# Sir-Teo/MuZero-Go

Hardware: AMD Instinct MI355X
Metric: MCTS simulations/sec (whole node) + self-play moves/sec, 9x9 Go, 200 sims/move (higher is better)
Workload: dtype fp32

## Files before the change

### muzero-go_amd/csrc/mzgo_capi.hip

```cpp
#include <hip/hip_runtime.h>

#include <algorithm>
#include <cmath>
#include <cstdarg>
#include <cstdio>
#include <cstring>
#include <map>
#include <string>
#include <vector>

#include "../../include/mzgo.h"
#include "mzgo_dispatch.hpp"
#include "mzgo_replay.hpp"
#include "mzgo_tower_host.hpp"
#include "mzgo_weights.hpp"

namespace mzgo {
extern const KernelSet kernels_n5_c96, kernels_n6_c96, kernels_n9_c96, kernels_n19_c96, kernels_n6_c128,
    kernels_n6_c64;

const KernelSet* find_kernels(int N, int C) {
  static const KernelSet* all[] = {&kernels_n5_c96, &kernels_n6_c96, &kernels_n9_c96, &kernels_n19_c96,
                                   &kernels_n6_c128, &kernels_n6_c64};
  for (const KernelSet* k : all)
// ... 38 lines not shown
  std::string key;
  std::vector<int64_t> shape;
};

std::vector<Spec> specs(int C, int A) {
  std::vector<Spec> out;
  for (int k = 0; k < WK_COUNT; ++k) {
    const WeightShape sh = weight_key_shape(k, C, A);
    out.push_back(Spec{kWeightKeyNames[k], std::vector<int64_t>(sh.d, sh.d + sh.nd)});
  }
  return out;
}

}

static int device_cus() {
  static int ncu[64];
  int dev = 0;
  if (hipGetDevice(&dev) != hipSuccess || dev < 0 || dev >= 64) return 0;
  if (ncu[dev] <= 0) {
    int n = 0;
    if (hipDeviceGetAttribute(&n, hipDeviceAttributeMultiprocessorCount, dev) != hipSuccess) n = 0;
    ncu[dev] = n;
  }
  return ncu[dev];
}

struct mzgo_engine {
  mzgo_config cfg;
  const KernelSet* ks = nullptr;
  int N = 0, C = 0, A = 0, CELLS = 0, CS = 0, G = 0, S = 0, M = 0;
  int TS = 0;
  std::map<std::string, std::vector<float>> sd;
  std::vector<Spec> spec;
  bool dirty = true;
  bool dev_weights = false;
  WeightLayout wl;
  float* d_w = nullptr;
  size_t d_w_bytes = 0;
  NetParams np{};
  EngineArrays E{};
  int* d_err = nullptr;
  unsigned* rq_head = nullptr;
  float* d_scr = nullptr;
  size_t scr_floats = 0;
  std::vector<void*> allocs;
  bool timing = false;
  std::vector<hipEvent_t> tev;
  int tn = 0;
  int64_t bytes = 0;
  int epoch = 0;
  int value_cache = 0;
  int arrival_conv = 1;
  const double* noise = nullptr;
  double* noise_out = nullptr;
  TowerHost* tower = nullptr;

  template <class T>
  int alloc(T** p, size_t n) {
    void* v = nullptr;
    hipError_t e = hipMalloc(&v, n * sizeof(T) + 256);
    if (e != hipSuccess) return fail(MZGO_EHIP, "hipMalloc(%zu): %s", n * sizeof(T), hipGetErrorString(e));
    allocs.push_back(v);
    bytes += (int64_t)(n * sizeof(T));
    *p = reinterpret_cast<T*>(v);
    return MZGO_OK;
  }
  ~mzgo_engine() {
    if (tower) {
      for (hipEvent_t ev : tower->evs) (void)hipEventDestroy(ev);
      tower->free_chains();
      for (void* p : {tower->d_wb, (void*)tower->d_wf, (void*)tower->ib, (void*)tower->ob, (void*)tower->s0,
                      (void*)tower->s1, (void*)tower->shp, (void*)tower->sact})
        if (p) (void)hipFree(p);
      if (tower->h_total) (void)hipHostFree(tower->h_total);
      tower->free_batch();
      delete tower;
    }
    for (hipEvent_t ev : tev) (void)hipEventDestroy(ev);
    for (void* p : allocs) (void)hipFree(p);
    if (d_w) (void)hipFree(d_w);
    if (d_scr) (void)hipFree(d_scr);
  }

  int ensure_blob() {
    if (d_w) return MZGO_OK;
    wl = weight_layout(N, C, A);
    HIPCHK(hipMalloc(&d_w, wl.total * 4));
    d_w_bytes = wl.total * 4;
    HIPCHK(hipMemset(d_w, 0, d_w_bytes));
    const float* b = d_w;
    const size_t* off = wl.off;
    np.w_conv1 = b + off[WP_CONV1_W]; np.b_conv1 = b + off[WP_CONV1_B];
    np.w_conv2 = b + off[WP_CONV2_W]; np.b_conv2 = b + off[WP_CONV2_B];
    np.w_conv3 = b + off[WP_CONV3_W]; np.b_conv3 = b + off[WP_CONV3_B];
    np.w_dyn = b + off[WP_DYN_W]; np.b_dyn = b + off[WP_DYN_B];
    np.emb = b + off[WP_EMB]; np.head_w = b + off[WP_HEAD_W]; np.etab = b + off[WP_ETAB];
    np.hs.reward_b = b + off[WP_REWARD_B]; np.hs.fc1_w = b + off[WP_FC1_W]; np.hs.fc1_b = b + off[WP_FC1_B];
    np.hs.fc2_w = b + off[WP_FC2_W]; np.hs.fc2_b = b + off[WP_FC2_B]; np.hs.value_b = b + off[WP_VALUE_B];
    np.hs.vfc_w = b + off[WP_VFC_W]; np.hs.vfc_b = b + off[WP_VFC_B]; np.hs.policy_b = b + off[WP_POLICY_B];
    np.hs.pass_logit = b + off[WP_PASS_LOGIT];
    return MZGO_OK;
  }

  int sync_weights() {
    if (C == 0) return fail(MZGO_EINVAL, "board-only engine (latent_dim 0) has no network");
    if (!dirty) return MZGO_OK;
    for (const Spec& s : spec)
      if (!sd.count(s.key)) return fail(MZGO_ENOWEIGHTS, "missing weight '%s'", s.key.c_str());
    if (tower) {
      HIPCHK(tower->upload(sd));
      dirty = false;
      return MZGO_OK;
    }
    if (int rc = ensure_blob()) return rc;
    const float* src[WK_COUNT];
    for (int k = 0; k < WK_COUNT; ++k) src[k] = sd[spec[k].key].data();
    std::vector<float> blob(wl.total, 0.f);
    pack_weights_host(wl, src, blob.data());
    HIPCHK(hipMemcpy(d_w, blob.data(), wl.total * 4, hipMemcpyHostToDevice));
    dev_weights = false;
    dirty = false;
    return MZGO_OK;
  }

  int tower_scratch(int B) {
    TowerHost& t = *tower;
    if (B <= t.scap) return MZGO_OK;
    for (void* p : {(void*)t.ib, (void*)t.ob, (void*)t.s0, (void*)t.s1, (void*)t.shp, (void*)t.sact})
      if (p) HIPCHK(hipFree(p));
    t.ib = t.ob = t.s0 = t.s1 = nullptr; t.shp = nullptr; t.sact = nullptr; t.scap = 0;
    const size_t n = (size_t)B * t.slot();
    for (bf16** q : {&t.ib, &t.ob, &t.s0, &t.s1}) {
      HIPCHK(hipMalloc((void**)q, n * sizeof(bf16)));
      HIPCHK(hipMemset(*q, 0, n * sizeof(bf16)));
    }
    HIPCHK(hipMalloc((void**)&t.shp, (size_t)B * t.CC * 3 * t.CS * sizeof(float)));
    HIPCHK(hipMalloc((void**)&t.sact, (size_t)B * sizeof(int)));
    t.scap = B;
    return MZGO_OK;
  }

  SearchParams search_params() const {
    SearchParams sp;
    sp.c_puct = cfg.c_puct; sp.discount = cfg.discount;
    sp.dirichlet_alpha = cfg.dirichlet_alpha; sp.dirichlet_epsilon = cfg.dirichlet_epsilon;
    sp.pass_epsilon = cfg.pass_epsilon; sp.num_simulations = S; sp.compat = cfg.compat;
    sp.variant = cfg.search_variant;
    sp.factored = cfg.direct_dynamics ? 0 : 1;
    sp.seed = cfg.seed;
    sp.helpers = 0;
    sp.net = 0;
    sp.tail = 0;
    const char* lz = getenv("MZGO_LAZY_ROWS");
    sp.lazy_rows = lz && atoi(lz) == 0 ? 0 : 1;
    sp.value_cache = value_cache;
    sp.arrival_conv = arrival_conv;
    sp.fast_simulations = 0;
    sp.full_search_prob = 1.0;
    return sp;
  }
  SearchParams selfplay_params() const {
    SearchParams sp = search_params();
    if (!tower && cfg.full_search_prob < 1.0) {
      sp.fast_simulations = cfg.fast_simulations;
      sp.full_search_prob = cfg.full_search_prob;
    }
    return sp;
  }
};

void mzgo::replay_engine_view(const mzgo_engine* e, ReplayEngineView* v) {
  const EngineArrays& E = e->E;
  *v = ReplayEngineView{e->N, e->G, e->M, e->C, e->tower ? 1 : 0, e->cfg.game_base, e->epoch,
                        E.stones, E.invd, E.meta, E.rec_stones, E.rec_invd, E.rec_flags, E.rec_action,
                        E.rec_value, E.rec_policy, E.rec_reward, E.final_reward};
}

extern "C" {

const char* mzgo_last_error(void) { return g_err.c_str(); }

void mzgo_default_config(mzgo_config* c, int N) {
  std::memset(c, 0, sizeof *c);
  c->board_size = N;
  c->latent_dim = 96;
  c->num_games = 1;
  c->num_simulations = 128;
  c->max_moves = N * N;
  c->compat = 0;
  c->temperature_moves = 15;
  c->c_puct = 2.5;
  c->discount = 0.99;
  c->dirichlet_alpha = 0.15;
  c->dirichlet_epsilon = 0.02;
  c->pass_epsilon = 0.01;
  c->temperature = 1.0;
  c->komi = 0.0;
  c->seed = 1234;
  c->fast_simulations = 0;
  c->full_search_prob = 1.0;
}

int mzgo_playout_budget_host(uint64_t seed, uint32_t key_gid, int move, int num_simulations, int fast_simulations,
                             double full_search_prob, int* budget) {
  if (!budget) return fail(MZGO_EINVAL, "mzgo_playout_budget_host: null budget");
  if (num_simulations < 1 || move < 0)
    return fail(MZGO_EINVAL, "mzgo_playout_budget_host: num_simulations %d must be >= 1 and move %d >= 0",
                num_simulations, move);
  if (fast_simulations < 0 || fast_simulations > num_simulations)
// ... 86 lines not shown
    T.bq_cap = t->bq_cap;
    chk(e->alloc(&T.pool, G * n1 * slot));
    chk(e->alloc(&t->t0, G * slot));
    chk(e->alloc(&t->t1, G * slot));
    chk(e->alloc(&T.rep_in, G * (size_t)t->P * 64));
    if (rc == MZGO_OK) {
      for (auto pr : {std::make_pair((void*)T.pool, G * n1 * slot), std::make_pair((void*)t->t0, G * slot),
                      std::make_pair((void*)t->t1, G * slot), std::make_pair((void*)T.rep_in, G * (size_t)t->P * 64)})
        if (hipMemset(pr.first, 0, pr.second * sizeof(bf16)) != hipSuccess) chk(fail(MZGO_EHIP, "hipMemset(tower) failed"));
    }
    T.slot = (long long)slot;
    chk(e->alloc(&T.hpart, G * (size_t)t->CC * 3 * e->CS));
    chk(e->alloc(&T.bq_n, G));
    chk(e->alloc(&T.bq_nid0, G));
    chk(e->alloc(&T.nbg, G));
    chk(e->alloc(&T.b_total, 1));
    if (rc == MZGO_OK && (hipMemset(T.bq_n, 0, G * sizeof(int)) != hipSuccess ||
                          hipHostMalloc(&t->h_total, sizeof(int), hipHostMallocDefault) != hipSuccess))
      chk(fail(MZGO_EHIP, "tower batch setup failed"));
    chk(e->alloc(&T.rootmask, G * A));
    chk(e->alloc(&T.passp, G));
    chk(e->alloc(&T.key, G));
    chk(e->alloc(&T.playing, G));
    chk(e->alloc(&T.evalact, G));
    chk(e->alloc(&T.in_idx, G));
    chk(e->alloc(&T.out_idx, G));
    chk(e->alloc(&T.root_idx, G));
    chk(e->alloc(&T.act, G));
    chk(e->alloc(&T.job, G * 3));
    chk(e->alloc(&T.simc, G));
    if (rc == MZGO_OK) {
      std::vector<int> ri(G);
      for (size_t g = 0; g < G; ++g) ri[g] = (int)(g * n1);
      if (hipMemcpy(T.root_idx, ri.data(), G * sizeof(int), hipMemcpyHostToDevice) != hipSuccess ||
          hipMemset(T.playing, 0, G * sizeof(int)) != hipSuccess || hipMemset(T.evalact, 0, G * sizeof(int)) != hipSuccess)
        chk(fail(MZGO_EHIP, "tower index setup failed"));
    }
  }
  if (C != 0) {
    chk(e->alloc(&E.prior, TSL * n1 * A));
    chk(e->alloc(&E.child, TSL * n1 * A));
    chk(e->alloc(&E.visits, TSL * n1));
    chk(e->alloc(&E.wsum, TSL * n1));
    chk(e->alloc(&E.root_prior, TSL * A));
    chk(e->alloc(&E.path, TSL * (n1 + 1)));
    chk(e->alloc(&E.nodes, TSL));
    chk(e->alloc(&E.nact, TSL * n1));
    const char* vc = getenv("MZGO_VALUE_CACHE");
    e->value_cache = !TW && !cfg->direct_dynamics && ks->value_cache_cap > 0 && e->S + 2 <= ks->value_cache_cap &&
                     !(vc && atoi(vc) == 0);
    if (e->value_cache) chk(e->alloc(&E.cval, TSL * n1 * A));
    const char* ac = getenv("MZGO_ARRIVAL_CONV");
    e->arrival_conv = !(ac && atoi(ac) <= 0);
    chk(e->alloc(&E.jobs, TSL * job_bytes(A)));
    chk(e->alloc(&E.mpq, 2 * (size_t)G + 1));
    chk(e->alloc(&E.rec_stones, G * M * CELLS));
    chk(e->alloc(&E.rec_invd, G * M * CELLS));
    chk(e->alloc(&E.rec_flags, G * M));
    chk(e->alloc(&E.rec_action, G * M));
    chk(e->alloc(&E.rec_value, G * M));
    chk(e->alloc(&E.rec_policy, G * M * A));
    chk(e->alloc(&E.rec_reward, G * M));
  }
  chk(e->alloc(&E.stones, G * CELLS));
  chk(e->alloc(&E.invd, G * CELLS));
  chk(e->alloc(&E.meta, G * 4));
  chk(e->alloc(&E.game_len, G));
  chk(e->alloc(&E.final_reward, G));
  chk(e->alloc(&E.status, G));
  chk(e->alloc(&E.counters, kCounters));
  chk(e->alloc(&e->d_err, 1));
  chk(e->alloc(&e->rq_head, 1));
#ifdef MZGO_STAMPS
  chk(e->alloc(&E.stamps, TSL * kStampPhases));
  if (E.stamps) (void)hipMemset(E.stamps, 0, TSL * kStampPhases * 8);
#endif
  if (rc != MZGO_OK) { delete e; return rc; }
  if (hipMemset(E.counters, 0, kCounters * sizeof(unsigned long long)) != hipSuccess ||
      hipMemset(e->d_err, 0, sizeof(int)) != hipSuccess) {
    delete e;
    return fail(MZGO_EHIP, "hipMemset failed");
  }
  hipError_t he = ks->board_reset(E, e->G, nullptr);
  if (he == hipSuccess) he = hipDeviceSynchronize();
  if (he != hipSuccess) { delete e; return fail(MZGO_EHIP, "board reset: %s", hipGetErrorString(he)); }
  *out = e;
  return MZGO_OK;
}

void mzgo_engine_destroy(mzgo_engine* e) { delete e; }

int64_t mzgo_engine_device_bytes(const mzgo_engine* e) { return e ? e->bytes + (int64_t)e->d_w_bytes : 0; }

int mzgo_set_weights(mzgo_engine* e, const char* key, const float* data, const int64_t* shape, int ndim) {
  if (!e || !key || !data || (!shape && ndim > 0)) return fail(MZGO_EINVAL, "null argument");
  for (const Spec& s : e->spec) {
    if (s.key != key) continue;
    if ((int)s.shape.size() != ndim) return fail(MZGO_EINVAL, "'%s': expected %zu dims, got %d", key, s.shape.size(), ndim);
    size_t n = 1;
    for (int i = 0; i < ndim; ++i) {
      if (shape[i] != s.shape[i])
        return fail(MZGO_EINVAL, "'%s': dim %d is %lld, expected %lld", key, i, (long long)shape[i], (long long)s.shape[i]);
      n *= (size_t)shape[i];
    }
    e->sd[key].assign(data, data + n);
    e->dirty = true;
// ... 578 lines not shown
```

### muzero-go_amd/csrc/mzgo_kernels.hpp

```cpp
#pragma once
#include "mzgo_jobs.hpp"
#include "mzgo_replay.hpp"

namespace mzgo {

template <class G>
constexpr bool rep_needs_scratch() {
  if constexpr (G::WINO) return Wino<G>::NSTRIP > 1;
  else return false;
}

struct NoRepJobs {
  __device__ bool operator()(int) const { return false; }
};

template <class G, class PlaneFn, class Jobs = NoRepJobs>
__device__ __forceinline__ void representation(Smem<G>& sm, const NetParams& np, PlaneFn planes, float* lat,
                                      int lat_stride, float* scr, unsigned long long* ts = nullptr,
                                      Jobs jobs = Jobs{}) {
  float* mid = rep_needs_scratch<G>() ? scr : lat;
  for (int i = tid_local(); i < 6 * G::CELLS; i += G::THREADS) {
    const int c = i / G::CELLS, j = i - c * G::CELLS;
    sm.u.in[c * G::CPAD + j] = planes(c, j);
  }
// ... 400 lines not shown
    if (y_lds_target<G>(sm) != nullptr && !shared_jobs<G>(sp)) load_hw<G>(sm, np.head_w);
    else load_y<G>(sm, pool, np.head_w);
    if (tid_local() == 0) { sm.t.npick = 0; sm.t.ngrab = 0; }
    __syncthreads();
    if (st) st->lap(61);
    if (shared_jobs<G>(sp)) {
      batch_expand_shared<G, Acc::LDS>(sm, np, sp, E, g, TV, K, 1, 0, sp.net, pool, el, n, 0, key, 0, nullptr, true);
    } else {
      if (wave_id() == 0) pick_sequence<G>(el, n, 0, K, key, 0, L.acts, &sm.t.npick, G::WAVES);
      batch_expand<G, Acc::LDS>(sm, np, sp, TV, K, 1, pool, st);
    }
    __syncthreads();
    if (st) st->lap(62);
    if (wave_id() == 0) {
      const int lane = lane_id_local();
      for (int k = lane; k < K; k += 64) {
        const int a = L.acts[k], nid = 1 + k;
        const double v = L.bv[k];
        T.init(nid);
        T.add(nid, v);
        T.set_child(0, a, nid);
        T.add_root_child(a, v);
        nact[nid] = a;
      }
      if (lane == 0) {
        const bool alt = sp.variant == 0;
        const double wroot = prefix_sums<G>(T.ws(0), L.bv, K, alt, nullptr);
        T.set(0, T.vis(0) + K, wroot);
        sm.t.newest = -1;
        sm.t.ycache = 0;
      }
    }
    __syncthreads();
    return K;
  }
}

template <class G, int DMAX>
struct VerifyLds {
  double cP[DMAX][64 * G::AP];
  double q[DMAX][64 * G::AP];
  double inv1n[DMAX][64 * G::AP];
  int n[DMAX][64 * G::AP];
  double qx[DMAX][G::A + 1], invr[DMAX][G::A + 1], sq[DMAX][G::A + 1], sx[DMAX][G::A + 1];
  uint64_t elig[DMAX][G::AP];
  double lo_o[DMAX], hi_o[DMAX];
  double cpx[DMAX];
  int x[DMAX], n0[DMAX], N0[DMAX];
  double wpre[DMAX][G::A + 9];
  double wroot[G::A + 9];
  uint64_t failm[G::AP];
  uint64_t exactm[DMAX][G::AP];
  int fail;
};
template <class G>
constexpr int verify_depth() { return G::AP > 2 ? 2 : 8; }
constexpr int kSeqK = 16, kSharedSeqK = 32;
__device__ __forceinline__ bool replay_sequential(int B, int depth) { return (B - 1) * (depth + 1) < kSeqK; }
__device__ __forceinline__ bool replay_parallel(bool shared, int B, int depth) {
  if (shared) return (B - 1) * (depth + 1) >= kSharedSeqK;
  return !replay_sequential(B, depth);
}

template <class G, class Acc, class V>
__device__ __forceinline__ void verify_load_level(Smem<G>& sm, const SearchParams& sp, const TreeView& TV,
                                                  const Acc& T, const int* nact, V& vl, int k, int l, int ract) {
  const int lane = lane_id_local();
  const int p = T.path(l);
  const int xa = l == 0 ? ract : nact[T.path(l + 1)];
  double lo = INFINITY, hi = -INFINITY, cpx = 0.0;
  int nx = 0;
#pragma unroll
  for (int j = 0; j < G::AP; ++j) {
    const int a = lane + 64 * j;
    const bool in = a < G::A;
    double P, w = 0.0;
    int n = 0;
    if (l == 0) {
      P = in ? T.root_prior(a) : 0.0;
      if constexpr (Acc::LDS) {
        if (in) { n = sm.t.rvis[a]; w = sm.t.rws[a]; }
      } else {
        const int c = in ? T.child(0, a) : -1;
        if (c >= 0) { n = T.vis(c); w = T.ws(c); }
      }
    } else {
      P = in ? (double)TV.prior[(size_t)p * G::A + a] : 0.0;
      const int c = in ? TV.child[(size_t)p * G::A + a] : -1;
      if (c >= 0) { n = T.vis(c); w = T.ws(c); }
    }
    const bool e = P > 0.0;
    const uint64_t el = __ballot(e);
    const double q = e ? (n > 0 ? ddiv(w, (double)n) : 0.0) : 0.0;
    const double cp = l == 0 ? sp.c_puct * P : (double)((float)sp.c_puct * (float)P);
    vl.cP[k][a] = cp;
    vl.q[k][a] = q;
    vl.inv1n[k][a] = 1.0 / (double)(1 + n);
    vl.n[k][a] = n;
    if (lane == 0) vl.elig[k][j] = el;
    if (e && a != xa) { lo = fmin_(lo, q); hi = fmax_(hi, q); }
    if (j == (xa >> 6)) {
      nx = __builtin_amdgcn_readlane(n, xa & 63);
      cpx = dpp::lane(cp, xa & 63);
    }
  }
  wave_minmax(lo, hi);
  if (lane == 0) {
    vl.lo_o[k] = lo;
    vl.hi_o[k] = hi;
    vl.x[k] = xa;
    vl.n0[k] = nx;
    vl.N0[k] = T.vis(p);
    vl.cpx[k] = cpx;
  }
}

template <class G, class Acc>
__device__ __forceinline__ void verify_levels(Smem<G>& sm, const SearchParams& sp, const TreeView& TV, const Acc& T,
                                              const int* nact, int D, int B, int l0, int nl, int ract,
                                              bool with_root, Stamp* st = nullptr, bool loaded = false,
                                              int BE = 0) {
  constexpr int DV = verify_depth<G>();
  typedef VerifyLds<G, DV> V;
  V& vl = *reinterpret_cast<V*>(&sm.u.f.wv[0]);
  const int wave = __builtin_amdgcn_readfirstlane(wave_id());
  const int lane = lane_id_local();
  const bool alt = sp.variant == 0;
  const double* bv = sm.u.f.bv;
  if (BE < B) BE = B;
  if (tid_local() < DV * G::AP) (&vl.exactm[0][0])[tid_local()] = 0;
  const int njobs = 2 * nl + (with_root ? 1 : 0);
  for (int job = wave; job < njobs; job += G::WAVES) {
    if (job == 2 * nl) {
      prefix_sums<G>(T.ws(0), bv, B, alt && ((D + 1) & 1), vl.wroot);
      continue;
    }
    if (job >= nl) {
      const int k = job - nl, l = l0 + k;
      prefix_sums<G>(T.ws(T.path(l + 1)), bv, B, alt && ((D - l) & 1), vl.wpre[k]);
      continue;
    }
    if (!loaded) verify_load_level<G, Acc>(sm, sp, TV, T, nact, vl, job, l0 + job, ract);
    if (st) st->lap(75);
  }
  __syncthreads();
  if (st) st->lap(76);
  for (int k = wave; k < nl; k += G::WAVES) {
    const int nx = vl.n0[k], N0 = vl.N0[k];
    const double lo = vl.lo_o[k], hi = vl.hi_o[k], cpx = vl.cpx[k];
#pragma unroll
    for (int j = 0; j < G::AP; ++j) {
      const int i = lane + 64 * j;
      bool bad = false;
      if (i <= B) {
        const int n1 = nx + i, Ni = N0 + i;
        const double qxi = n1 > 0 ? ddiv(vl.wpre[k][i], (double)n1) : 0.0;
        const double loi = fmin_(lo, qxi), hii = fmax_(hi, qxi);
        const double sqi = dsqrt((double)(sp.variant == 1 ? Ni + 1 : (Ni > 1 ? Ni : 1)));
        const double sxi = (hii > loi ? ddiv(qxi - loi, hii - loi) : qxi) + ddiv(cpx * sqi, (double)(1 + n1));
        vl.qx[k][i] = qxi;
        vl.invr[k][i] = hii > loi ? 1.0 / (hii - loi) : 0.0;
        vl.sq[k][i] = sqi;
        vl.sx[k][i] = sxi;
        bad = i >= 1 && i < BE && !(sxi > -INFINITY);
      }
      const uint64_t bb = __ballot(bad);
      if (lane == 0 && bb) atomicOr(reinterpret_cast<unsigned long long*>(&vl.failm[j]), (unsigned long long)bb);
    }
    if (st) st->lap(77);
  }
  __syncthreads();
  if (st) st->lap(72);
  const unsigned long long ts0 = st ? st->now() : 0;
  for (int k = 0; k < nl; ++k) {
    const int xa = vl.x[k];
    const double lo_o = vl.lo_o[k], hi_o = vl.hi_o[k];
    double loi[G::AP], invr[G::AP], sqi[G::AP], sxi[G::AP], tol[G::AP];
    bool spread[G::AP];
    uint64_t beaten[G::AP], close[G::AP];
#pragma unroll
    for (int j = 0; j < G::AP; ++j) {
      const int i = lane + 64 * j;
      const int ii = i <= B ? i : B;
      const double qxi = vl.qx[k][ii];
      loi[j] = fmin_(lo_o, qxi);
      spread[j] = fmax_(hi_o, qxi) > loi[j];
      invr[j] = vl.invr[k][ii];
      sqi[j] = vl.sq[k][ii];
      sxi[j] = vl.sx[k][ii];
      tol[j] = 1e-12 * (1.0 + fabs(sxi[j]));
      beaten[j] = 0;
      close[j] = 0;
    }
    constexpr int KW = (G::A + G::WAVES - 1) / G::WAVES;
    static_assert(KW <= 64, "one lane per child of the wave");
    const int amine = wave + G::WAVES * lane;
    const bool mine = lane < KW && amine < G::A && amine != xa &&
                      ((vl.elig[k][(amine < G::A ? amine : 0) >> 6] >> (amine & 63)) & 1ull);
    const int ac = mine ? amine : 0;
    const double qa_l = vl.q[k][ac], cpa_l = vl.cP[k][ac], ia_l = vl.inv1n[k][ac];
    const uint64_t todo = __ballot(mine);
    for (uint64_t mm = todo; mm; mm &= mm - 1) {
      const int kk = __builtin_ctzll(mm);
      const double qa = dpp::lane(qa_l, kk), cpa = dpp::lane(cpa_l, kk), ia = dpp::lane(ia_l, kk);
#pragma unroll
      for (int j = 0; j < G::AP; ++j) {
        if (64 * j >= BE) break;
        const double sc = (spread[j] ? (qa - loi[j]) * invr[j] : qa) + (cpa * sqi[j]) * ia;
        beaten[j] |= __ballot(sc > sxi[j] + tol[j]);
        close[j] |= __ballot(!(fabs(sc - sxi[j]) > tol[j]));
      }
    }
    if (lane == 0) {
#pragma unroll
      for (int j = 0; j < G::AP; ++j) {
        if (beaten[j]) atomicOr(reinterpret_cast<unsigned long long*>(&vl.failm[j]), (unsigned long long)beaten[j]);
        if (close[j] & ~beaten[j])
          atomicOr(reinterpret_cast<unsigned long long*>(&vl.exactm[k][j]), (unsigned long long)(close[j] & ~beaten[j]));
      }
    }
  }
  if (st) st->wave_add(80, st->now() - ts0);
  __syncthreads();
  if (st) st->lap(78);
  for (int k = 0; k < nl; ++k) {
    uint64_t open[G::AP];
#pragma unroll
    for (int j = 0; j < G::AP; ++j) {
      const uint64_t o = vl.exactm[k][j] & ~vl.failm[j];
      open[j] = ((uint64_t)__builtin_amdgcn_readfirstlane((uint32_t)(o >> 32)) << 32) |
                __builtin_amdgcn_readfirstlane((uint32_t)o);
    }
    int c = 0;
#pragma unroll
    for (int j = 0; j < G::AP; ++j) {
      for (uint64_t mm = open[j]; mm; mm &= mm - 1, ++c) {
        if (c % G::WAVES != wave) continue;
        const int i = 64 * j + __builtin_ctzll(mm);
        if (i < 1 || i >= BE) continue;
        const int xa = vl.x[k];
        const int nx = vl.n0[k] + i;
        const double qx = vl.qx[k][i];
        const double lo = fmin_(vl.lo_o[k], qx), hi = fmax_(vl.hi_o[k], qx);
        const double sq = vl.sq[k][i], sx = vl.sx[k][i];
        uint64_t beat = 0;
#pragma unroll
        for (int jj = 0; jj < G::AP; ++jj) {
          const int a = lane + 64 * jj;
          const bool el = (vl.elig[k][jj] >> lane) & 1ull;
          const bool isx = a == xa;
          const double q = isx ? qx : vl.q[k][a];
          const int n = isx ? nx : vl.n[k][a];
          const double qn = hi > lo ? ddiv(q - lo, hi - lo) : q;
          const double sc = qn + ddiv(vl.cP[k][a] * sq, (double)(1 + n));
          beat |= __ballot(el && !isx && (sc > sx || (sc == sx && a < xa)));
        }
        if (beat && lane == 0)
          atomicOr(reinterpret_cast<unsigned long long*>(&vl.failm[i >> 6]), 1ull << (i & 63));
      }
    }
  }
  __syncthreads();
  if (st) st->lap(79);
}

struct VerifyPlan {
  int gs, ngroups, g0;
  bool shared;
};
template <class G, class Acc>
__device__ __forceinline__ VerifyPlan verify_plan(const SearchParams& sp, int D) {
  constexpr int DV = verify_depth<G>();
  VerifyPlan v;
  v.gs = D <= 4 ? 1 : DV;
  v.ngroups = (D + v.gs - 1) / v.gs;
  v.shared = !Acc::LDS && shared_jobs<G>(sp) && v.ngroups > 1;
  if (!v.shared) { v.gs = DV; v.ngroups = (D + DV - 1) / DV; }
  v.g0 = D < v.gs ? D : v.gs;
  return v;
}

template <class G, class Acc>
__device__ __forceinline__ void verify_preload(Smem<G>& sm, const SearchParams& sp, const TreeView& TV, const Acc& T,
                                               const int* nact, int D) {
  if constexpr (decltype(sm.u.f)::BATCH) {
    typedef VerifyLds<G, verify_depth<G>()> V;
    V& vl = *reinterpret_cast<V*>(&sm.u.f.wv[0]);
    const VerifyPlan v = verify_plan<G, Acc>(sp, D);
    for (int k = __builtin_amdgcn_readfirstlane(wave_id()); k < v.g0; k += G::WAVES)
      verify_load_level<G, Acc>(sm, sp, TV, T, nact, vl, k, k, sm.t.ract);
  }
}

template <class G, class Acc>
__device__ __forceinline__ int replay_share(Smem<G>& sm, const SearchParams& sp, const TreeView& TV, const Acc& T,
                                            const int* nact, const JobView& J, const JobInfo& I, unsigned bseq,
                                            Stamp* st = nullptr, bool preloaded = false) {
  typedef VerifyLds<G, verify_depth<G>()> V;
  V& vl = *reinterpret_cast<V*>(&sm.u.f.wv[0]);
  const int gs = I.group(), D = I.depth;
  int mine = 0;
  if (preloaded) {
    verify_levels<G, Acc>(sm, sp, TV, T, nact, D, I.batch, 0, min(gs, D), I.act, false, st, true);
    ++mine;
  }
  for (int grp; (grp = job_claim(sm, J, bseq, I.units, 1)) >= 0; ++mine)
    verify_levels<G, Acc>(sm, sp, TV, T, nact, D, I.batch, grp * gs, min(gs, D - grp * gs), I.act, false, st);
  if (mine > 0 && tid_local() < G::AP && vl.failm[tid_local()])
    __hip_atomic_fetch_or(J.h->failm + tid_local(), (unsigned long long)vl.failm[tid_local()], __ATOMIC_RELAXED,
                          __HIP_MEMORY_SCOPE_AGENT);
  return mine;
}
template <class G>
__device__ __forceinline__ int replay_help(Smem<G>& sm, const SearchParams& sp, const EngineArrays& E, int g,
                                           const TreeView& TV, const JobView& J, const JobInfo& I, unsigned bseq) {
  typedef VerifyLds<G, verify_depth<G>()> V;
  V& vl = *reinterpret_cast<V*>(&sm.u.f.wv[0]);
  const double* bvg = J.bv(G::A);
  for (int k = tid_local(); k < I.batch; k += G::THREADS) sm.u.f.bv[k] = bvg[k];
  if (tid_local() < G::AP) vl.failm[tid_local()] = 0;
  __syncthreads();
  const TreeAcc<G, false> T(TV, sm.t);
  return replay_share<G, TreeAcc<G, false>>(sm, sp, TV, T, E.nact + (size_t)g * ((size_t)E.S + 1), J, I, bseq);
}

template <class G, class Acc>
__device__ __forceinline__ int verify_batch(Smem<G>& sm, const SearchParams& sp, const EngineArrays& E, int g,
                                            const TreeView& TV, Acc& T, int* nact, int leaf, int D, int B, int nid,
                                            Stamp* st = nullptr, bool preloaded = false, bool ext = false,
                                            bool* resume = nullptr, bool yleaf_lds = true) {
  if constexpr (!decltype(sm.u.f)::BATCH) {
    return 0;
  } else {
  constexpr int DV = verify_depth<G>();
  typedef VerifyLds<G, DV> V;
  static_assert(sizeof(V) <= sizeof(sm.u.f.wv), "verification arrays overlay the batch buffers");
  V& vl = *reinterpret_cast<V*>(&sm.u.f.wv[0]);
  const int lane = lane_id_local();
  const bool alt = sp.variant == 0;
  const double* bv = sm.u.f.bv;
  if (tid_local() < G::AP) vl.failm[tid_local()] = 0;
  const VerifyPlan vp = verify_plan<G, Acc>(sp, D);
  if (vp.shared) {
    const JobView J = job_of<G>(E, g);
    const JobInfo I = job_info(kJobReplay, vp.ngroups, nid, leaf, vp.gs, sm.t.ract, D, B);
    const unsigned bseq = job_post(J, I, preloaded ? 1u : 0u, [&](unsigned) {
      if (tid_local() < G::AP)
        __hip_atomic_store(J.h->failm + tid_local(), 0ull, __ATOMIC_RELAXED, __HIP_MEMORY_SCOPE_AGENT);
    });
    const int mine = replay_share<G, Acc>(sm, sp, TV, T, nact, J, I, bseq, st, preloaded);
    asm volatile("s_waitcnt vmcnt(0)" ::: "memory");
    __syncthreads();
    job_wait(J, mine, I.units);
    if (tid_local() < G::AP)
      vl.failm[tid_local()] = __hip_atomic_load(J.h->failm + tid_local(), __ATOMIC_RELAXED, __HIP_MEMORY_SCOPE_AGENT);
  } else {
    for (int l0 = 0; l0 < D; l0 += DV)
      verify_levels<G, Acc>(sm, sp, TV, T, nact, D, B, l0, D - l0 < DV ? D - l0 : DV, sm.t.ract, l0 == 0, st,
                            preloaded && l0 == 0, ext ? B + 1 : B);
  }
  if ((D == 0 || vp.shared) && tid_local() == 0) prefix_sums<G>(T.ws(0), bv, B, alt && ((D + 1) & 1), vl.wroot);
  if (tid_local() == 0) {
    int f = 64 * G::AP;
#pragma unroll
    for (int j = G::AP - 1; j >= 0; --j) {
      uint64_t mm = vl.failm[j];
      if (j == 0) mm &= ~1ull;
      if (mm) f = 64 * j + __builtin_ctzll(mm);
    }
    vl.fail = f < B ? f : (ext && !vp.shared && f > B ? B + 1 : B);
  }
  __syncthreads();
  if (st) st->lap(73);
  const int m = vl.fail < B ? vl.fail : B;
  if (resume) *resume = vl.fail > B;
  if (wave_id() == 0) {
    for (int d = lane; d <= D; d += 64) {
      if (d == 0) {
        T.set(0, T.vis(0) + m, vl.wroot[m]);
      } else {
        const int p = T.path(d);
        const bool neg = alt && ((D + 1 - d) & 1);
        double w = T.ws(p);
#pragma unroll 8
        for (int k = 0; k < m; ++k) w = w + (neg ? -bv[k] : bv[k]);
        const int n = T.vis(p) + m;
        T.set(p, n, w);
        if constexpr (Acc::LDS)
          if (d == 1) { sm.t.rvis[sm.t.ract] = n; sm.t.rws[sm.t.ract] = w; }
      }
    }
    wave_lds_sync();
    for (int i = lane; i < m; i += 64) {
      const int ai = sm.u.f.acts[i], n2 = nid + i;
      const double v = 0.0 + bv[i];
      T.set(n2, 1, v);
      nact[n2] = ai;
      T.set_child(leaf, ai, n2);
      if (leaf == 0) T.add_root_child(ai, v);
    }
    if (lane == 0) { sm.t.newest = -1; if (yleaf_lds) sm.t.ycache = leaf; }
  }
  __syncthreads();
  if (st) st->lap(74);
  return m;
  }
}

template <class G, class Acc>
__device__ __forceinline__ void sim_loop(Smem<G>& sm, const NetParams& np, const SearchParams& sp,
                                         const EngineArrays& E, int g, const TreeView& TV, uint64_t key) {
  float* pool = pool_of<G>(E, g);
  const size_t node_floats = (size_t)G::C * G::CS;
  float* scratch = pool + (size_t)(E.S + 1) * node_floats;
  int* nact = E.nact + (size_t)g * ((size_t)E.S + 1);
  const int S = sp.num_simulations;
  const bool factored = sp.factored != 0;
  constexpr bool BATCH = decltype(sm.u.f)::BATCH;
  Acc T(TV, sm.t);
  tree_reset_root<G>(T);
  if (tid_local() == 0) {
    sm.t.newest = -1; sm.t.newp_node = -1; sm.t.ycache = -1; sm.t.rowc_node = -1; sm.t.lognode = -1;
  }
  __syncthreads();

  int nodes = 1, convs = 0;
  constexpr bool VCACHE = Acc::LDS && BATCH && decltype(sm.u.f)::CACHE;
  const bool vcache = VCACHE && factored && sp.value_cache != 0 && E.cval != nullptr && !shared_jobs<G>(sp);
  int nbcomp = 0, nbcache = 0, ncut = 0;
  constexpr bool ARRIVAL = Acc::LDS && BATCH && G::WINO && decltype(sm.u.f)::CACHE && Wino<G>::NSTRIP == 1;
  const bool arrival = ARRIVAL && factored && sp.arrival_conv != 0 && sp.variant == 0 && !sp.tail &&
                       !shared_jobs<G>(sp);
  int narr_lds = 0, narr_l2 = 0;
  auto cache_cut = [&](int leaf, int m, int B) {
    double* cv = E.cval + ((size_t)g * ((size_t)E.S + 1) + (size_t)leaf) * G::A;
    for (int i = m + tid_local() - 64; tid_local() >= 64 && i < B; i += G::THREADS - 64)
      cv[sm.u.f.acts[i]] = sm.u.f.bv[i];
    if (tid_local() == 0) sm.t.cvm[leaf >> 5] |= 1u << (leaf & 31);
    __syncthreads();
  };
  int rows = 0;
  const bool eager_rows = !(Acc::LDS || shared_jobs<G>(sp) || (decltype(sm.u.f)::GLOBAL_Y && sp.lazy_rows));
  Stamp st(E.stamps);
  int sim = 0;
  if (factored) {
    sim = root_batch<G, Acc>(sm, np, sp, E, g, TV, T, pool, scratch, nact, key, &st);
    if (eager_rows) rows += sim;
    nodes += sim;
    convs += sim > 0 ? 1 : 0;
    st.lap(4);
  }
  bool pending = false;
  int node0 = 0, depth0 = 0;
  while (sim < S) {
    if (!pending) {
      if (wave_id() == 0) {
        const int a = select_leaf<G>(sm.t, T, sp, key, sim, &st, node0, depth0);
        if (lane_id_local() == 0) sm.t.action = a;
// ... 914 lines not shown
```

### muzero-go_amd/csrc/mzgo_search.hpp

```cpp
#pragma once
#include "mzgo_common.hpp"
#include <type_traits>

namespace mzgo {

struct SearchParams {
  double c_puct;
  double discount;
  double dirichlet_alpha;
  double dirichlet_epsilon;
  double pass_epsilon;
  int num_simulations;
  int compat;
  int variant;
  int factored;
  uint64_t seed;
  int helpers;
  int net;
  int tail;
  int lazy_rows;
  int value_cache;
  int arrival_conv;
  int fast_simulations;
  double full_search_prob;
};

__host__ __device__ __forceinline__ int playout_budget(uint64_t key, int S, int F, double p) {
  if (F == 0) return S;
  return u01(draw(key, TAG_BUDGET, 0)) < p ? S : F;
}
__host__ __device__ __forceinline__ int playout_budget(const SearchParams& sp, uint32_t kid, int mv) {
  return playout_budget(stream_key(sp.seed, kid, (uint32_t)mv), sp.num_simulations, sp.fast_simulations,
                        sp.full_search_prob);
}

struct TreeView {
  float* prior;
  int* child;
  int* visits;
  double* wsum;
  double* root_prior;
  int* path;
};

constexpr int kRawRow = -2;
constexpr int kLazyRow = -3;
constexpr int kNeedLogits = -4;

template <class G>
struct TreeLds {
  float logits[G::A];
  float fbuf[G::A];
  double dbuf[G::A];
  uint8_t valid[G::A];
  double pass_prior;
  float reward, value;
  int leaf, action, nid, depth, nodes, bcast;
  int yready;
  int npick;
  int ngrab;
  int nunexp;
  uint64_t umask[G::AP];
  int ycache;
  int lognode;
  int lpar, lact;
  float hsc[56];
  int svis[G::TREE_CAP > 0 ? G::TREE_CAP : 1];
  double sws[G::TREE_CAP > 0 ? G::TREE_CAP : 1];
  int spath[G::TREE_CAP > 0 ? G::TREE_CAP : 1];
  int rchild[G::TREE_CAP > 0 ? G::A : 1];
  double rprior[G::TREE_CAP > 0 ? G::A : 1];
  int rvis[G::TREE_CAP > 0 ? G::A : 1];
  double rws[G::TREE_CAP > 0 ? G::A : 1];
  int ract;
  int rowc_node;
// ... 876 lines not shown
```

Measured before the change: 144.7 million.

## Trim replay verification: packed child screening, skip idle exact pass, drop barrier

Splits the replay verification into helpers and adds a replay_trim mode, on by default at level 4. For small batches the child screening packs two or four children per wave iteration instead of one. The exact tie-check pass and its barrier are skipped when no level has open candidates. At the top level, wave 0 computes the fail index itself instead of waiting on a block barrier, and reuses the stored prefix sums for path updates. This cuts block-wide syncs and wasted lanes in the speculative-replay check, at the cost of more code paths whose tie-handling and prefix-sum reuse must stay exactly equivalent.

```diff
diff --git a/muzero-go_amd/csrc/mzgo_capi.hip b/muzero-go_amd/csrc/mzgo_capi.hip
--- a/muzero-go_amd/csrc/mzgo_capi.hip
+++ b/muzero-go_amd/csrc/mzgo_capi.hip
@@ -114,6 +114,7 @@
   int epoch = 0;
   int value_cache = 0;
   int arrival_conv = 1;
+  int replay_trim = 4;
   const double* noise = nullptr;
   double* noise_out = nullptr;
   TowerHost* tower = nullptr;
@@ -218,6 +219,7 @@
     sp.lazy_rows = lz && atoi(lz) == 0 ? 0 : 1;
     sp.value_cache = value_cache;
     sp.arrival_conv = arrival_conv;
+    sp.replay_trim = replay_trim;
     sp.fast_simulations = 0;
     sp.full_search_prob = 1.0;
     return sp;
@@ -410,6 +412,9 @@
     if (e->value_cache) chk(e->alloc(&E.cval, TSL * n1 * A));
     const char* ac = getenv("MZGO_ARRIVAL_CONV");
     e->arrival_conv = !(ac && atoi(ac) <= 0);
+    const char* rt = getenv("MZGO_REPLAY_TRIM");
+    const int rtv = rt ? atoi(rt) : 4;
+    e->replay_trim = rt && rt[0] == '0' && rtv == 0 ? 0 : rtv == 2 || rtv == 3 ? rtv : 4;
     chk(e->alloc(&E.jobs, TSL * job_bytes(A)));
     chk(e->alloc(&E.mpq, 2 * (size_t)G + 1));
     chk(e->alloc(&E.rec_stones, G * M * CELLS));
diff --git a/muzero-go_amd/csrc/mzgo_kernels.hpp b/muzero-go_amd/csrc/mzgo_kernels.hpp
--- a/muzero-go_amd/csrc/mzgo_kernels.hpp
+++ b/muzero-go_amd/csrc/mzgo_kernels.hpp
@@ -476,6 +476,7 @@
   uint64_t failm[G::AP];
   uint64_t exactm[DMAX][G::AP];
   int fail;
+  unsigned open;
 };
 template <class G>
 constexpr int verify_depth() { return G::AP > 2 ? 2 : 8; }
@@ -539,6 +540,168 @@
   }
 }
 
+template <class G, class V>
+__device__ __forceinline__ void verify_score_level(const SearchParams& sp, V& vl, int k, int B, int BE,
+                                                   uint64_t* bad) {
+  const int lane = lane_id_local();
+  const int nx = vl.n0[k], N0 = vl.N0[k];
+  const double lo = vl.lo_o[k], hi = vl.hi_o[k], cpx = vl.cpx[k];
+#pragma unroll
+  for (int j = 0; j < G::AP; ++j) {
+    const int i = lane + 64 * j;
+    bool b = false;
+    if (i <= B) {
+      const int n1 = nx + i, Ni = N0 + i;
+      const double qxi = n1 > 0 ? ddiv(vl.wpre[k][i], (double)n1) : 0.0;
+      const double loi = fmin_(lo, qxi), hii = fmax_(hi, qxi);
+      const double sqi = dsqrt((double)(sp.variant == 1 ? Ni + 1 : (Ni > 1 ? Ni : 1)));
+      const double sxi = (hii > loi ? ddiv(qxi - loi, hii - loi) : qxi) + ddiv(cpx * sqi, (double)(1 + n1));
+      vl.qx[k][i] = qxi;
+      vl.invr[k][i] = hii > loi ? 1.0 / (hii - loi) : 0.0;
+      vl.sq[k][i] = sqi;
+      vl.sx[k][i] = sxi;
+      b = i >= 1 && i < BE && !(sxi > -INFINITY);
+    }
+    bad[j] = __ballot(b);
+  }
+}
+
+struct ScreenCol {
+  double loi, invr, sqi, sxi, tol;
+  bool spread;
+};
+template <class V>
+__device__ __forceinline__ ScreenCol screen_col(const V& vl, int k, int i, int B) {
+  const int ii = i <= B ? i : B;
+  const double qxi = vl.qx[k][ii];
+  ScreenCol c;
+  c.loi = fmin_(vl.lo_o[k], qxi);
+  c.spread = fmax_(vl.hi_o[k], qxi) > c.loi;
+  c.invr = vl.invr[k][ii];
+  c.sqi = vl.sq[k][ii];
+  c.sxi = vl.sx[k][ii];
+  c.tol = 1e-12 * (1.0 + fabs(c.sxi));
+  return c;
+}
+__device__ __forceinline__ double screen_score(const ScreenCol& c, double qa, double cpa, double ia) {
+  return (c.spread ? (qa - c.loi) * c.invr : qa) + (cpa * c.sqi) * ia;
+}
+template <class G, class V>
+__device__ __forceinline__ uint64_t screen_children(const V& vl, int k, int wave, bool& mine) {
+  constexpr int KW = (G::A + G::WAVES - 1) / G::WAVES;
+  static_assert(KW <= 64, "one lane per child of the wave");
+  const int lane = lane_id_local();
+  const int amine = wave + G::WAVES * lane;
+  mine = lane < KW && amine < G::A && amine != vl.x[k] &&
+         ((vl.elig[k][(amine < G::A ? amine : 0) >> 6] >> (amine & 63)) & 1ull);
+  return __ballot(mine);
+}
+template <class G, class V>
+__device__ __forceinline__ void screen_wide(const V& vl, int k, int wave, int B, int BE, uint64_t* beaten,
+                                            uint64_t* close) {
+  const int lane = lane_id_local();
+  ScreenCol col[G::AP];
+#pragma unroll
+  for (int j = 0; j < G::AP; ++j) {
+    col[j] = screen_col(vl, k, lane + 64 * j, B);
+    beaten[j] = 0;
+    close[j] = 0;
+  }
+  bool mine;
+  const uint64_t todo = screen_children<G>(vl, k, wave, mine);
+  const int ac = mine ? wave + G::WAVES * lane : 0;
+  const double qa_l = vl.q[k][ac], cpa_l = vl.cP[k][ac], ia_l = vl.inv1n[k][ac];
+  for (uint64_t mm = todo; mm; mm &= mm - 1) {
+    const int kk = __builtin_ctzll(mm);
+    const double qa = dpp::lane(qa_l, kk), cpa = dpp::lane(cpa_l, kk), ia = dpp::lane(ia_l, kk);
+#pragma unroll
+    for (int j = 0; j < G::AP; ++j) {
+      if (64 * j >= BE) break;
+      const double sc = screen_score(col[j], qa, cpa, ia);
+      beaten[j] |= __ballot(sc > col[j].sxi + col[j].tol);
+      close[j] |= __ballot(!(fabs(sc - col[j].sxi) > col[j].tol));
+    }
+  }
+}
+template <class G, int P, class V>
+__device__ __forceinline__ void screen_packed(const V& vl, int k, int wave, int B, uint64_t* beaten,
+                                              uint64_t* close) {
+  constexpr int W = 64 / P;
+  static_assert(P == 2 || P == 4, "two or four children per iteration");
+  const int lane = lane_id_local();
+  const int c = lane / W;
+  const ScreenCol col = screen_col(vl, k, lane & (W - 1), B);
+  bool mine;
+  uint64_t mm = screen_children<G>(vl, k, wave, mine);
+  uint64_t bt = 0, cl = 0;
+  while (mm) {
+    int kk = -1;
+#pragma unroll
+    for (int cc = 0; cc < P; ++cc) {
+      const int t = mm ? __builtin_ctzll(mm) : -1;
+      mm &= mm - 1;
+      if (c == cc) kk = t;
+    }
+    const bool have = kk >= 0;
+    const int a = wave + G::WAVES * (have ? kk : 0);
+    const double sc = screen_score(col, vl.q[k][a], vl.cP[k][a], vl.inv1n[k][a]);
+    bt |= __ballot(have && sc > col.sxi + col.tol);
+    cl |= __ballot(have && !(fabs(sc - col.sxi) > col.tol));
+  }
+  auto fold = [](uint64_t b) __attribute__((always_inline)) {
+    b |= b >> 32;
+    if (P == 4) b |= b >> 16;
+    return b & ((1ull << W) - 1);
+  };
+#pragma unroll
+  for (int j = 0; j < G::AP; ++j) { beaten[j] = 0; close[j] = 0; }
+  beaten[0] = fold(bt);
+  close[0] = fold(cl);
+}
+
+template <class G, class V>
+__device__ __forceinline__ void verify_exact(V& vl, int nl, int BE, int wave) {
+  const int lane = lane_id_local();
+  for (int k = 0; k < nl; ++k) {
+    uint64_t open[G::AP];
+#pragma unroll
+    for (int j = 0; j < G::AP; ++j) {
+      const uint64_t o = vl.exactm[k][j] & ~vl.failm[j];
+      open[j] = ((uint64_t)__builtin_amdgcn_readfirstlane((uint32_t)(o >> 32)) << 32) |
+                __builtin_amdgcn_readfirstlane((uint32_t)o);
+    }
+    int c = 0;
+#pragma unroll
+    for (int j = 0; j < G::AP; ++j) {
+      for (uint64_t mm = open[j]; mm; mm &= mm - 1, ++c) {
+        if (c % G::WAVES != wave) continue;
+        const int i = 64 * j + __builtin_ctzll(mm);
+        if (i < 1 || i >= BE) continue;
+        const int xa = vl.x[k];
+        const int nx = vl.n0[k] + i;
+        const double qx = vl.qx[k][i];
+        const double lo = fmin_(vl.lo_o[k], qx), hi = fmax_(vl.hi_o[k], qx);
+        const double sq = vl.sq[k][i], sx = vl.sx[k][i];
+        uint64_t beat = 0;
+#pragma unroll
+        for (int jj = 0; jj < G::AP; ++jj) {
+          const int a = lane + 64 * jj;
+          const bool el = (vl.elig[k][jj] >> lane) & 1ull;
+          const bool isx = a == xa;
+          const double q = isx ? qx : vl.q[k][a];
+          const int n = isx ? nx : vl.n[k][a];
+          const double qn = hi > lo ? ddiv(q - lo, hi - lo) : q;
+          const double sc = qn + ddiv(vl.cP[k][a] * sq, (double)(1 + n));
+          beat |= __ballot(el && !isx && (sc > sx || (sc == sx && a < xa)));
+        }
+        if (beat && lane == 0)
+          atomicOr(reinterpret_cast<unsigned long long*>(&vl.failm[i >> 6]), 1ull << (i & 63));
+      }
+    }
+  }
+}
+
+constexpr int kTrimAll = 4;
 template <class G, class Acc>
 __device__ __forceinline__ void verify_levels(Smem<G>& sm, const SearchParams& sp, const TreeView& TV, const Acc& T,
                                               const int* nact, int D, int B, int l0, int nl, int ract,
@@ -551,8 +714,12 @@
   const int lane = lane_id_local();
   const bool alt = sp.variant == 0;
   const double* bv = sm.u.f.bv;
+  const int trim = Acc::LDS ? sp.replay_trim : 0;
   if (BE < B) BE = B;
+  BE = __builtin_amdgcn_readfirstlane(BE);
+  static_assert(DV * G::AP < G::THREADS, "a thread per word to zero");
   if (tid_local() < DV * G::AP) (&vl.exactm[0][0])[tid_local()] = 0;
+  if (trim >= 3 && tid_local() == DV * G::AP) vl.open = 0;
   const int njobs = 2 * nl + (with_root ? 1 : 0);
   for (int job = wave; job < njobs; job += G::WAVES) {
     if (job == 2 * nl) {
@@ -570,121 +737,43 @@
   __syncthreads();
   if (st) st->lap(76);
   for (int k = wave; k < nl; k += G::WAVES) {
-    const int nx = vl.n0[k], N0 = vl.N0[k];
-    const double lo = vl.lo_o[k], hi = vl.hi_o[k], cpx = vl.cpx[k];
-#pragma unroll
-    for (int j = 0; j < G::AP; ++j) {
-      const int i = lane + 64 * j;
-      bool bad = false;
-      if (i <= B) {
-        const int n1 = nx + i, Ni = N0 + i;
-        const double qxi = n1 > 0 ? ddiv(vl.wpre[k][i], (double)n1) : 0.0;
-        const double loi = fmin_(lo, qxi), hii = fmax_(hi, qxi);
-        const double sqi = dsqrt((double)(sp.variant == 1 ? Ni + 1 : (Ni > 1 ? Ni : 1)));
-        const double sxi = (hii > loi ? ddiv(qxi - loi, hii - loi) : qxi) + ddiv(cpx * sqi, (double)(1 + n1));
-        vl.qx[k][i] = qxi;
-        vl.invr[k][i] = hii > loi ? 1.0 / (hii - loi) : 0.0;
-        vl.sq[k][i] = sqi;
-        vl.sx[k][i] = sxi;
-        bad = i >= 1 && i < BE && !(sxi > -INFINITY);
-      }
-      const uint64_t bb = __ballot(bad);
-      if (lane == 0 && bb) atomicOr(reinterpret_cast<unsigned long long*>(&vl.failm[j]), (unsigned long long)bb);
-    }
+    uint64_t bad[G::AP];
+    verify_score_level<G>(sp, vl, k, B, BE, bad);
+#pragma unroll
+    for (int j = 0; j < G::AP; ++j)
+      if (lane == 0 && bad[j])
+        atomicOr(reinterpret_cast<unsigned long long*>(&vl.failm[j]), (unsigned long long)bad[j]);
     if (st) st->lap(77);
   }
   __syncthreads();
   if (st) st->lap(72);
   const unsigned long long ts0 = st ? st->now() : 0;
+  bool anyopen = false;
   for (int k = 0; k < nl; ++k) {
-    const int xa = vl.x[k];
-    const double lo_o = vl.lo_o[k], hi_o = vl.hi_o[k];
-    double loi[G::AP], invr[G::AP], sqi[G::AP], sxi[G::AP], tol[G::AP];
-    bool spread[G::AP];
     uint64_t beaten[G::AP], close[G::AP];
-#pragma unroll
-    for (int j = 0; j < G::AP; ++j) {
-      const int i = lane + 64 * j;
-      const int ii = i <= B ? i : B;
-      const double qxi = vl.qx[k][ii];
-      loi[j] = fmin_(lo_o, qxi);
-      spread[j] = fmax_(hi_o, qxi) > loi[j];
-      invr[j] = vl.invr[k][ii];
-      sqi[j] = vl.sq[k][ii];
-      sxi[j] = vl.sx[k][ii];
-      tol[j] = 1e-12 * (1.0 + fabs(sxi[j]));
-      beaten[j] = 0;
-      close[j] = 0;
-    }
-    constexpr int KW = (G::A + G::WAVES - 1) / G::WAVES;
-    static_assert(KW <= 64, "one lane per child of the wave");
-    const int amine = wave + G::WAVES * lane;
-    const bool mine = lane < KW && amine < G::A && amine != xa &&
-                      ((vl.elig[k][(amine < G::A ? amine : 0) >> 6] >> (amine & 63)) & 1ull);
-    const int ac = mine ? amine : 0;
-    const double qa_l = vl.q[k][ac], cpa_l = vl.cP[k][ac], ia_l = vl.inv1n[k][ac];
-    const uint64_t todo = __ballot(mine);
-    for (uint64_t mm = todo; mm; mm &= mm - 1) {
-      const int kk = __builtin_ctzll(mm);
-      const double qa = dpp::lane(qa_l, kk), cpa = dpp::lane(cpa_l, kk), ia = dpp::lane(ia_l, kk);
+    if (trim >= 2 && BE <= 16) screen_packed<G, 4>(vl, k, wave, B, beaten, close);
+    else if (trim >= 2 && BE <= 32) screen_packed<G, 2>(vl, k, wave, B, beaten, close);
+    else screen_wide<G>(vl, k, wave, B, BE, beaten, close);
+    if (lane == 0) {
 #pragma unroll
       for (int j = 0; j < G::AP; ++j) {
-        if (64 * j >= BE) break;
-        const double sc = (spread[j] ? (qa - loi[j]) * invr[j] : qa) + (cpa * sqi[j]) * ia;
-        beaten[j] |= __ballot(sc > sxi[j] + tol[j]);
-        close[j] |= __ballot(!(fabs(sc - sxi[j]) > tol[j]));
-      }
-    }
-    if (lane == 0) {
-#pragma unroll
-      for (int j = 0; j < G::AP; ++j) {
-        if (beaten[j]) atomicOr(reinterpret_cast<unsigned long long*>(&vl.failm[j]), (unsigned long long)beaten[j]);
-        if (close[j] & ~beaten[j])
-          atomicOr(reinterpret_cast<unsigned long long*>(&vl.exactm[k][j]), (unsigned long long)(close[j] & ~beaten[j]));
-      }
-    }
-  }
+        const uint64_t fl = beaten[j], op = close[j] & ~beaten[j];
+        if (fl) atomicOr(reinterpret_cast<unsigned long long*>(&vl.failm[j]), (unsigned long long)fl);
+        if (op) atomicOr(reinterpret_cast<unsigned long long*>(&vl.exactm[k][j]), (unsigned long long)op);
+        const int nb = BE - 64 * j;
+        const uint64_t live = (nb >= 64 ? ~0ull : nb > 0 ? (1ull << nb) - 1 : 0ull) & (j == 0 ? ~1ull : ~0ull);
+        if (trim >= 3) anyopen |= (op & live) != 0;
+      }
+    }
+  }
+  if (lane == 0 && anyopen) atomicOr(&vl.open, 1u);
   if (st) st->wave_add(80, st->now() - ts0);
   __syncthreads();
   if (st) st->lap(78);
-  for (int k = 0; k < nl; ++k) {
-    uint64_t open[G::AP];
-#pragma unroll
-    for (int j = 0; j < G::AP; ++j) {
-      const uint64_t o = vl.exactm[k][j] & ~vl.failm[j];
-      open[j] = ((uint64_t)__builtin_amdgcn_readfirstlane((uint32_t)(o >> 32)) << 32) |
-                __builtin_amdgcn_readfirstlane((uint32_t)o);
-    }
-    int c = 0;
-#pragma unroll
-    for (int j = 0; j < G::AP; ++j) {
-      for (uint64_t mm = open[j]; mm; mm &= mm - 1, ++c) {
-        if (c % G::WAVES != wave) continue;
-        const int i = 64 * j + __builtin_ctzll(mm);
-        if (i < 1 || i >= BE) continue;
-        const int xa = vl.x[k];
-        const int nx = vl.n0[k] + i;
-        const double qx = vl.qx[k][i];
-        const double lo = fmin_(vl.lo_o[k], qx), hi = fmax_(vl.hi_o[k], qx);
-        const double sq = vl.sq[k][i], sx = vl.sx[k][i];
-        uint64_t beat = 0;
-#pragma unroll
-        for (int jj = 0; jj < G::AP; ++jj) {
-          const int a = lane + 64 * jj;
-          const bool el = (vl.elig[k][jj] >> lane) & 1ull;
-          const bool isx = a == xa;
-          const double q = isx ? qx : vl.q[k][a];
-          const int n = isx ? nx : vl.n[k][a];
-          const double qn = hi > lo ? ddiv(q - lo, hi - lo) : q;
-          const double sc = qn + ddiv(vl.cP[k][a] * sq, (double)(1 + n));
-          beat |= __ballot(el && !isx && (sc > sx || (sc == sx && a < xa)));
-        }
-        if (beat && lane == 0)
-          atomicOr(reinterpret_cast<unsigned long long*>(&vl.failm[i >> 6]), 1ull << (i & 63));
-      }
-    }
-  }
-  __syncthreads();
+  if (trim < 3 || __builtin_amdgcn_readfirstlane(vl.open) != 0) {
+    verify_exact<G>(vl, nl, BE, wave);
+    __syncthreads();
+  }
   if (st) st->lap(79);
 }
 
@@ -784,7 +873,7 @@
                             preloaded && l0 == 0, ext ? B + 1 : B);
   }
   if ((D == 0 || vp.shared) && tid_local() == 0) prefix_sums<G>(T.ws(0), bv, B, alt && ((D + 1) & 1), vl.wroot);
-  if (tid_local() == 0) {
+  auto fail_index = [&]() __attribute__((always_inline)) {
     int f = 64 * G::AP;
 #pragma unroll
     for (int j = G::AP - 1; j >= 0; --j) {
@@ -792,22 +881,39 @@
       if (j == 0) mm &= ~1ull;
       if (mm) f = 64 * j + __builtin_ctzll(mm);
     }
-    vl.fail = f < B ? f : (ext && !vp.shared && f > B ? B + 1 : B);
-  }
-  __syncthreads();
-  if (st) st->lap(73);
-  const int m = vl.fail < B ? vl.fail : B;
-  if (resume) *resume = vl.fail > B;
+    return f < B ? f : (ext && !vp.shared && f > B ? B + 1 : B);
+  };
+  const bool trim4 = Acc::LDS && sp.replay_trim >= kTrimAll;
+  int fail = 0;
+  if (trim4) {
+    if (wave_id() == 0) {
+      wave_lds_sync();
+      fail = fail_index();
+      if (lane == 0) vl.fail = fail;
+    }
+  } else {
+    if (tid_local() == 0) vl.fail = fail_index();
+    __syncthreads();
+    if (st) st->lap(73);
+    fail = vl.fail;
+  }
+  const int m = fail < B ? fail : B;
+  const bool sums_kept = trim4 && !vp.shared && D <= DV;
   if (wave_id() == 0) {
     for (int d = lane; d <= D; d += 64) {
       if (d == 0) {
         T.set(0, T.vis(0) + m, vl.wroot[m]);
       } else {
         const int p = T.path(d);
-        const bool neg = alt && ((D + 1 - d) & 1);
-        double w = T.ws(p);
+        double w;
+        if (sums_kept) {
+          w = vl.wpre[d - 1][m];
+        } else {
+          const bool neg = alt && ((D + 1 - d) & 1);
+          w = T.ws(p);
 #pragma unroll 8
-        for (int k = 0; k < m; ++k) w = w + (neg ? -bv[k] : bv[k]);
+          for (int k = 0; k < m; ++k) w = w + (neg ? -bv[k] : bv[k]);
+        }
         const int n = T.vis(p) + m;
         T.set(p, n, w);
         if constexpr (Acc::LDS)
@@ -826,8 +932,10 @@
     if (lane == 0) { sm.t.newest = -1; if (yleaf_lds) sm.t.ycache = leaf; }
   }
   __syncthreads();
+  const int failed = vl.fail;
+  if (resume) *resume = failed > B;
   if (st) st->lap(74);
-  return m;
+  return failed < B ? failed : B;
   }
 }
 
diff --git a/muzero-go_amd/csrc/mzgo_search.hpp b/muzero-go_amd/csrc/mzgo_search.hpp
--- a/muzero-go_amd/csrc/mzgo_search.hpp
+++ b/muzero-go_amd/csrc/mzgo_search.hpp
@@ -21,6 +21,7 @@
   int lazy_rows;
   int value_cache;
   int arrival_conv;
+  int replay_trim;
   int fast_simulations;
   double full_search_prob;
 };
```

Result: no change. 146.0 million, median of 6 (+0.9%).
